# jarek1992/raytracer_project

Hardware: AMD Instinct MI355X
Metric: Msamples/sec (rays·bounces) (higher is better)
Workload: dtype f64

## Files before the change

### raytracer_project_amd/csrc/zr_build.hip

```cpp
#include <cstring>
#include <hip/hip_runtime.h>
#include <rocprim/device/device_radix_sort.hpp>
#include <rocprim/device/device_scan.hpp>
#include <rocprim/iterator/counting_iterator.hpp>
#include <rocprim/iterator/transform_iterator.hpp>

#include <algorithm>
#include <chrono>
#include <cstdio>
#include <vector>

#include "zr_build.h"
#include "zr_bvh.h"

namespace zr {
namespace {

constexpr uint32_t NONE = 0xFFFFFFFFu;
constexpr int MAX_R = 32;
constexpr uint32_t M_KIND = 7u, M_UNIFORM = 8u, M_LEAF = 16u;

struct PBox { float lo[3]; uint32_t kind; float hi[3]; uint32_t pad; };
struct Cl { float lo[3]; uint32_t node; float hi[3]; uint32_t pad; };
struct BNode { float lo[3]; uint32_t left; float hi[3]; uint32_t right; };
// ... 346 lines not shown
    const uint32_t p = parent[id];
    if (p != NONE && (nmeta[p] & M_LEAF)) return;
    leaf_pos[id] = out.base[nmeta[id] & M_KIND] + rank[leaf_pos[id]];
}

__device__ __forceinline__ void plane_sum(float origin, float scale, int q, double& s, double& e) {
    const double a = (double)origin, m = (double)q * (double)scale;
    s = a + m;
    const double bb = s - a;
    e = (a - (s - bb)) + (m - bb);
}
__device__ __forceinline__ bool plane_le(float origin, float scale, int q, double x) { double s, e; plane_sum(origin, scale, q, s, e); return s < x || (s == x && e <= 0.0); }
__device__ __forceinline__ bool plane_ge(float origin, float scale, int q, double x) { double s, e; plane_sum(origin, scale, q, s, e); return s > x || (s == x && e >= 0.0); }
__device__ __forceinline__ double plane_val(float origin, float scale, int q) { return (double)origin + (double)q * (double)scale; }

__device__ bool quant_axis(const float* lo, const float* hi, int n, float& origin, float& scale, uint32_t* qlo, uint32_t* qhi) {
    float mn = lo[0], mx = hi[0];
    for (int k = 1; k < n; k++) { mn = fminf(mn, lo[k]); mx = fmaxf(mx, hi[k]); }
    if (!(fabsf(mn) <= 1e30f) || !(fabsf(mx) <= 1e30f)) return false;
    origin = nextafterf(mn, -__builtin_huge_valf());
    const double ext = (double)mx - (double)origin;
    int e = ext > 0 ? (int)ceil(log2(ext / 255.0)) : -100;
    const int emin = origin != 0.0f ? max(-100, ilogbf(origin) - 30) : -100;
    if (e < emin) e = emin;
    for (int tries = 0; tries < 64; tries++, e++) {
        scale = ldexpf(1.0f, e);
        bool ok = true;
        for (int k = 0; k < n && ok; k++) {
            long ql = (long)floor(((double)lo[k] - (double)origin) / (double)scale);
            ql = ql < 0 ? 0 : (ql > 255 ? 255 : ql);
            while (ql > 0 && !plane_le(origin, scale, (int)ql, (double)lo[k])) ql--;
            if (!plane_le(origin, scale, (int)ql, (double)lo[k])) ok = false;
            long qh = (long)ceil(((double)hi[k] - (double)origin) / (double)scale);
            qh = qh < 0 ? 0 : (qh > 255 ? 255 : qh);
            while (qh < 255 && !plane_ge(origin, scale, (int)qh, (double)hi[k])) qh++;
            if (!plane_ge(origin, scale, (int)qh, (double)hi[k])) ok = false;
            qlo[k] = (uint32_t)ql; qhi[k] = (uint32_t)qh;
        }
        if (ok) return true;
    }
    return false;
}

__device__ bool quantise(const BNode* __restrict__ bn, const uint32_t* kids, int nk, NodeQ& nq, float& worst) {
    uint32_t ql[3][4], qh[3][4];
    for (int k = 0; k < 6; k++) nq.q[k] = 0;
    for (int ax = 0; ax < 3; ax++) {
        float lo[4], hi[4];
        for (int k = 0; k < nk; k++) { lo[k] = bn[kids[k]].lo[ax]; hi[k] = bn[kids[k]].hi[ax]; }
        if (!quant_axis(lo, hi, nk, nq.origin[ax], nq.scale[ax], ql[ax], qh[ax])) return false;
        for (int k = 0; k < nk; k++) { nq.q[ax] |= ql[ax][k] << (8 * k); nq.q[3 + ax] |= qh[ax][k] << (8 * k); }
    }
    worst = 1;
    for (int k = 0; k < nk; k++) {
        double d[3];
        for (int ax = 0; ax < 3; ax++) d[ax] = plane_val(nq.origin[ax], nq.scale[ax], (int)qh[ax][k]) - plane_val(nq.origin[ax], nq.scale[ax], (int)ql[ax][k]);
        const double aq = d[0] * d[1] + d[1] * d[2] + d[2] * d[0];
        const BNode b = bn[kids[k]];
        const double at = (double)half_area(b.lo, b.hi);
        const float rr = at > 0 ? (float)(aq / at) : (aq > 0 ? 3.0e38f : 1.0f);
        if (!(rr <= worst)) worst = rr;
    }
    return true;
}

struct PlanOut {
    uint32_t counter;
    uint32_t quant_fail;
    uint32_t quad_depth;
    uint32_t kept_closed;
    uint32_t root_demand;
    uint32_t pad_[3];
    NodeF root;
};

__device__ __forceinline__ uint32_t leaf_ref(const uint32_t* __restrict__ nmeta, const uint32_t* __restrict__ ncount, const uint32_t* __restrict__ leaf_pos, uint32_t node) {
    return ZR_REF_LEAF | ((nmeta[node] & M_KIND) << 28) | ((ncount[node] - 1u) << 24) | leaf_pos[node];
}

__global__ __launch_bounds__(256) void k_plan(const BNode* __restrict__ bn, const uint32_t* __restrict__ nmeta, const uint32_t* __restrict__ ncount,
                                              const uint32_t* __restrict__ leaf_pos, uint32_t node_lo, uint32_t node_hi, uint32_t root, int root_in_array, float open_ratio,
                                              const zr_object* __restrict__ objs, const uint32_t* __restrict__ run_demand,
                                              uint32_t* __restrict__ qroot, uint32_t* __restrict__ qlevel, uint32_t* __restrict__ qinst, NodeQ* __restrict__ quads,
                                              PlanOut* __restrict__ po) {
    const uint32_t id = node_lo + blockIdx.x * 256 + threadIdx.x;
    if (id >= node_hi) return;
    const bool is_root = id == root;
    const bool fp32_root = is_root && !root_in_array;
    const uint32_t me = qroot[id];
    if (!fp32_root && me == NONE) return;
    uint32_t kids[4]; int nk = 0;
    NodeQ nq;
    for (int ax = 0; ax < 3; ax++) { nq.origin[ax] = 0; nq.scale[ax] = 1; }
    for (int k = 0; k < 6; k++) nq.q[k] = 0;
    float worst = 1;
    if (nmeta[id] & M_LEAF) {
        kids[nk++] = id;
        if (!fp32_root && !quantise(bn, kids, nk, nq, worst)) atomicExch(&po->quant_fail, 1u);
    } else {
        const BNode b = bn[id];
        kids[0] = b.left; kids[1] = b.right; nk = 2;
        if (!fp32_root && !quantise(bn, kids, nk, nq, worst)) atomicExch(&po->quant_fail, 1u);
        while (nk < 4) {
            int best = -1; float ba = -1;
            for (int k = 0; k < nk; k++) {
                if (nmeta[kids[k]] & M_LEAF) continue;
                const BNode c = bn[kids[k]];
                const float ar = half_area(c.lo, c.hi);
                if (ar > ba) { ba = ar; best = k; }
            }
            if (best < 0) break;
            uint32_t trial[4];
            for (int k = 0; k < nk; k++) trial[k] = kids[k];
            const BNode ob = bn[kids[best]];
            trial[best] = ob.left; trial[nk] = ob.right;
            if (!fp32_root) {
                NodeQ tq = nq; float w = 1;
                if (!quantise(bn, trial, nk + 1, tq, w)) { atomicExch(&po->quant_fail, 1u); break; }
                if (w > open_ratio && w > worst) { atomicAdd(&po->kept_closed, 1u); break; }
                nq = tq; worst = w;
            }
            for (int k = 0; k <= nk; k++) kids[k] = trial[k];
            nk++;
        }
    }
    int n_inner = 0;
    for (int k = 0; k < nk; k++) if (!(nmeta[kids[k]] & M_LEAF)) n_inner++;
    uint32_t next = n_inner ? atomicAdd(&po->counter, (uint32_t)n_inner) : 0u;
    const uint32_t my_level = fp32_root ? 0u : qlevel[me];
    uint32_t refs[4] = {ZR_REF_EMPTY, ZR_REF_EMPTY, ZR_REF_EMPTY, ZR_REF_EMPTY};
    uint32_t inst_demand = 0;
    for (int k = 0; k < nk; k++) {
        const uint32_t c = kids[k];
        if (nmeta[c] & M_LEAF) {
            refs[k] = leaf_ref(nmeta, ncount, leaf_pos, c);
            if ((nmeta[c] & M_KIND) == ZR_KIND_INSTANCE && run_demand && objs) {
                uint32_t q = c;
                while (bn[q].right != NONE) q = bn[q].left;
// ... 229 lines not shown

}

DeviceBuilder::~DeviceBuilder() {
    if (arena_) (void)hipFree(arena_);
    for (void* p : keep_) (void)hipFree(p);
}
void* DeviceBuilder::alloc_keep(size_t bytes) {
    void* p = nullptr;
    if (hipMalloc(&p, bytes < 64 ? 64 : bytes) != hipSuccess) { (void)hipGetLastError(); return nullptr; }
    keep_.push_back(p);
    return p;
}
size_t DeviceBuilder::scratch_bytes(uint32_t n) {
    const size_t N = 2 * (size_t)n + 2;
    return (size_t)n * (32 + 16 + 8 + 64 + 4 + 1 + 4 + 1 + 4 + 4 + 4 + 4 + 4 + 4 + 8) + N * (32 + 4 + 4 + 4 + 4 + 4 + 4) + (size_t)n * 24 + (64u << 20);
}
hipError_t DeviceBuilder::reserve(size_t bytes) {
    if (bytes <= arena_bytes_) return hipSuccess;
    if (arena_) { (void)hipStreamSynchronize(st_); (void)hipFree(arena_); arena_ = nullptr; arena_bytes_ = 0; }
    hipError_t e = hipMalloc((void**)&arena_, bytes);
    if (e != hipSuccess) { (void)hipGetLastError(); err_ = "out of device memory for the build's scratch"; return e; }
    arena_bytes_ = bytes;
    return hipSuccess;
}

hipError_t DeviceBuilder::build(const BuildSceneIn& in, const zr_object* d_objects, const uint8_t* d_code, uint32_t first_triangle, uint32_t n,
                                const BuildParams& bp, bool root_in_array, const BuildPrimOut& out, const uint32_t* d_run_demand, uint32_t depth_limit,
                                bool stats, BuiltTree& t) {
    hipError_t e;
    err_ = ""; use_host_ = false;
    if (n == 0) { err_ = "empty tree"; use_host_ = true; return hipErrorInvalidValue; }
    Params prm;
    prm.ct = bp.ct; prm.max_leaf = bp.max_leaf < 1 ? 1 : (bp.max_leaf > 16 ? 16 : bp.max_leaf); prm.open_ratio = bp.open_ratio;
    prm.radius = bp.radius < 1 ? 1 : (bp.radius > MAX_R ? MAX_R : bp.radius);
    for (int k = 0; k < 8; k++) { prm.ck[k] = bp.ck[k]; prm.cap[k] = bp.leaf_cap[k]; }
    const size_t N = 2 * (size_t)n;
    const uint32_t nb_max = (n + 255) / 256;
    PBox* pbox; uint64_t *keys_a, *keys_b; uint32_t *vals_a, *vals_b; Cl *cl_a, *cl_b; BNode* bn;
    uint32_t *parent, *ncount, *nmeta, *leaf_pos, *qroot, *nn, *blk_keep, *blk_new, *keep_off, *new_off, *dfs_obj, *rank, *scanned, *qlevel, *qinst, *qdem, *compound, *state;
    float* ncost; uint8_t *act, *dfs_kind; PlanOut* po; void* tmp; size_t tmp_bytes = 0;
    uint32_t *qinst_plan, *qmap, *qscan; NodeQ* quads_plan;
    auto layout = [&](unsigned char* base) -> size_t {
        unsigned char* at = base;
        auto take = [&](size_t bytes) { void* p = at; at += (bytes + 255) / 256 * 256; return p; };
        pbox = (PBox*)take((size_t)n * sizeof(PBox));
        keys_a = (uint64_t*)take((size_t)n * 8); keys_b = (uint64_t*)take((size_t)n * 8);
        vals_a = (uint32_t*)take((size_t)n * 4); vals_b = (uint32_t*)take((size_t)n * 4);
        cl_a = (Cl*)take((size_t)n * sizeof(Cl)); cl_b = (Cl*)take((size_t)n * sizeof(Cl));
        bn = (BNode*)take(N * sizeof(BNode));
        parent = (uint32_t*)take(N * 4); ncount = (uint32_t*)take(N * 4); nmeta = (uint32_t*)take(N * 4);
        ncost = (float*)take(N * 4);
        leaf_pos = (uint32_t*)take(N * 4); qroot = (uint32_t*)take(N * 4);
        nn = (uint32_t*)take((size_t)n * 4); act = (uint8_t*)take(n);
        blk_keep = (uint32_t*)take((size_t)nb_max * 4); blk_new = (uint32_t*)take((size_t)nb_max * 4);
        keep_off = (uint32_t*)take((size_t)nb_max * 4); new_off = (uint32_t*)take((size_t)nb_max * 4);
        dfs_obj = (uint32_t*)take((size_t)n * 4); dfs_kind = (uint8_t*)take(n);
        rank = (uint32_t*)take((size_t)n * 4); scanned = (uint32_t*)take((size_t)n * 4);
        qlevel = (uint32_t*)take((size_t)n * 4); qinst = (uint32_t*)take((size_t)n * 4); qdem = (uint32_t*)take((size_t)n * 4);
        qinst_plan = (uint32_t*)take((size_t)n * 4); qmap = (uint32_t*)take((size_t)n * 4); qscan = (uint32_t*)take(N * 4);
        quads_plan = (NodeQ*)take((size_t)n * sizeof(NodeQ));
        compound = (uint32_t*)take((size_t)n * 8);
        state = (uint32_t*)take(256);
        po = (PlanOut*)take(sizeof(PlanOut));
        if (tmp_bytes == 0) {
            size_t a = 0, b = 0, c = 0;
            (void)rocprim::radix_sort_pairs(nullptr, a, keys_a, keys_b, vals_a, vals_b, (size_t)n, 0, 63, st_);
            (void)rocprim::exclusive_scan(nullptr, b, rocprim::make_transform_iterator(dfs_kind, IsKind{0}), scanned, 0u, (size_t)n, rocprim::plus<uint32_t>(), st_);
// ... 143 lines not shown
    if ((e = hipMemsetAsync(qinst, 0, (size_t)n * 4, st_)) != hipSuccess) return e;
    if ((e = hipMemsetAsync(qdem, 0, (size_t)n * 4, st_)) != hipSuccess) return e;
    auto renumber = [&]() -> hipError_t {
        auto flags = rocprim::make_transform_iterator(rocprim::make_counting_iterator<uint32_t>(0u), QRootFlag{qroot, root});
        hipError_t er = rocprim::exclusive_scan(tmp, tmp_bytes, flags, qscan, 0u, (size_t)n_nodes, rocprim::plus<uint32_t>(), st_);
        if (er != hipSuccess) { err_ = "scan failed"; return er; }
        hipLaunchKernelGGL(k_qmap, grid_for(n_nodes), dim3(256), 0, st_, qroot, qscan, n_nodes, qmap);
        hipLaunchKernelGGL(k_qpermute, grid_for(quad_cap), dim3(256), 0, st_, quads_plan, quads, qinst_plan, qinst, qmap, quad_cap, po);
        return hipSuccess;
    };
    if (root_in_array) {
        if ((e = hipMemsetAsync(qroot + root, 0, 4, st_)) != hipSuccess) return e;
        if ((e = hipMemsetAsync(qlevel, 0, 4, st_)) != hipSuccess) return e;
    }
    if (n == 1) {
        hipLaunchKernelGGL(k_plan, dim3(1), dim3(256), 0, st_, bn, nmeta, ncount, leaf_pos, root, root + 1, root, root_in_array ? 1 : 0, prm.open_ratio, d_objects, d_run_demand,
                           qroot, qlevel, qinst_plan, quads_plan, po);
        if ((e = renumber()) != hipSuccess) return e;
        hipLaunchKernelGGL(k_demand, dim3(1), dim3(256), 0, st_, qroot, root, root + 1, root, root_in_array ? 1 : 0, quads, qinst, qdem, po);
    } else {
        for (size_t b = batch_start.size() - 1; b-- > 0;) {
            const uint32_t lo = batch_start[b], hi = batch_start[b + 1];
            hipLaunchKernelGGL(k_plan, grid_for(hi - lo), dim3(256), 0, st_, bn, nmeta, ncount, leaf_pos, lo, hi, root, root_in_array ? 1 : 0, prm.open_ratio, d_objects,
                               d_run_demand, qroot, qlevel, qinst_plan, quads_plan, po);
        }
        if ((e = renumber()) != hipSuccess) return e;
        for (size_t b = 0; b + 1 < batch_start.size(); b++) {
            const uint32_t lo = batch_start[b], hi = batch_start[b + 1];
            hipLaunchKernelGGL(k_demand, grid_for(hi - lo), dim3(256), 0, st_, qroot, lo, hi, root, root_in_array ? 1 : 0, quads, qinst, qdem, po);
        }
    }
    lap(4);
    uint32_t n_pairs = 1;
    if (n >= 2) {
        uint32_t h_root_meta = 0;
        if ((e = hipMemcpyAsync(&h_root_meta, nmeta + root, 4, hipMemcpyDeviceToHost, st_)) != hipSuccess) return e;
        if ((e = hipStreamSynchronize(st_)) != hipSuccess) return e;
        if (h_root_meta & M_LEAF) hipLaunchKernelGGL(k_pair_leaf_root, dim3(1), dim3(1), 0, st_, bn, nmeta, ncount, leaf_pos, root, pairs);
// ... 44 lines not shown
```

### raytracer_project_amd/csrc/zr_commit.cpp

```cpp
#include "zr_flatten.h"

namespace {

int finish_commit(zr_scene* s, const CommitSummary& cs, size_t n_objs) {
    int rc;
    if (std::getenv("ZR_QUANT_STATS")) std::fprintf(stderr, "[zr] 4-wide nodes: %zu quantised (64 B) + FP32 root; %zu children kept closed for the grid\n", cs.n_quads, cs.kept_closed);
    s->quad_ok = cs.quant_ok && cs.n_quads < (1u << 31) && cs.max_leaf <= 16 && cs.n_sph < (1u << 24) && cs.n_tri < (1u << 24) && cs.n_cube < (1u << 24) &&
                 cs.n_media < (1u << 24) && cs.n_wrapped < (1u << 24) && cs.n_pcube < (1u << 24) && cs.n_insts < (1u << 24);
    if ((rc = s->d_ops.upload(s->ops.data(), s->ops.size()))) return rc;
    {
        std::vector<zr_material> mats = s->materials;
        auto tex_uses_uv = [&](uint32_t id) {
            std::vector<uint32_t> todo{id}; int guard = 0;
            while (!todo.empty() && guard++ < 4096) {
                uint32_t t = todo.back(); todo.pop_back();
                if (t >= s->textures.size()) continue;
                const zr_texture& tx = s->textures[t];
                if (tx.kind >= ZR_TEX_IMAGE_U8) return true;
                if (tx.kind == ZR_TEX_CHECKER) { todo.push_back(tx.odd); todo.push_back(tx.even); }
            }
            return guard >= 4096;
        };
        for (zr_material& m : mats) m.pad_ = (m.bump_tex != ZR_NO_TEXTURE || (m.kind != ZR_MAT_DIELECTRIC && tex_uses_uv(m.tex))) ? 1u : 0u;
        if ((rc = s->d_mats.upload(mats))) return rc;
// ... 215 lines not shown
            hipError_t e = builder->build(in, nullptr, nullptr, grp.first_triangle, grp.triangle_count, bp, true, go, nullptr, ZR_STACK_DEPTH - 2, false, runs[g]);
            if (e != hipSuccess) return build_fail(e);
            for (int k = 0; k < 6; k++) gbox[g * 6 + k] = runs[g].box[k];
            run_demand[g] = runs[g].demand;
        }
    }
    if (ng) { if ((rc = r_gbox.upload(gbox)) || (rc = d_run_demand.upload(run_demand))) return rc; in.group_box = r_gbox.p; }
    phase("groups' trees");
    zr::BuiltTree world;
    world.want_boxes = std::getenv("ZR_BUILD_CHECK") != nullptr;
    {
        hipError_t e = builder->build(in, r_objs.p, r_code.p, 0, n, bp, false, out, ng ? d_run_demand.p : nullptr, ZR_STACK_DEPTH - 2, commit_stats, world);
        if (e != hipSuccess) return build_fail(e);
    }
    if (commit_stats)
        std::fprintf(stderr, "[zr] device build: boxes+keys %.2f, sort %.2f, PLOC %.2f (%u iterations), order %.2f, 4-wide %.2f, pairs %.2f, emit %.2f ms; depth %u, %u pairs, %u quads\n",
                     world.ms[0], world.ms[1], world.ms[2], world.ploc_iterations, world.ms[3], world.ms[4], world.ms[5], world.ms[6], world.depth, world.n_pairs, world.n_quads);
    if (world.want_boxes) {
        std::vector<zr::BuildBox> gb(ng);
        for (size_t g = 0; g < ng; g++) for (int k = 0; k < 3; k++) { gb[g].lo[k] = gbox[g * 6 + k]; gb[g].hi[k] = gbox[g * 6 + 3 + k]; }
        Boxer boxer{*s, &gb};
        size_t bad = 0;
        for (uint32_t k = 0; k < n; k++) {
            const zr::BuildBox hb = boxer.chain(objs[k].type, objs[k].index, objs[k].chain_first, objs[k].chain_count);
            const float* d = &world.dbg_boxes[(size_t)k * 8];
            bool ok = true;
            for (int a = 0; a < 3; a++) if (!((double)d[a] <= hb.lo[a]) || !((double)d[4 + a] >= hb.hi[a])) ok = false;
            if (!ok && bad++ < 8)
                std::fprintf(stderr, "[zr] BUILD_CHECK: object %u (type %u, chain %u): device box [%g %g %g | %g %g %g] does not contain the host's [%g %g %g | %g %g %g]\n", k, objs[k].type,
                             objs[k].chain_count, d[0], d[1], d[2], d[4], d[5], d[6], hb.lo[0], hb.lo[1], hb.lo[2], hb.hi[0], hb.hi[1], hb.hi[2]);
        }
        if (bad) return fail(ZR_E_DEVICE, "ZR_BUILD_CHECK: %zu of %u object boxes computed on the device do not contain the host's", bad, n);
// ... 290 lines not shown
                    env_double("ZR_BVH_COST_MEDIUM", 3.0), env_double("ZR_BVH_COST_WRAPPED", 3.0), env_double("ZR_BVH_COST_PCUBE", 1.5),
                    env_double("ZR_BVH_COST_GROUP", 16.0), 1};
    int max_leaf = (int)env_double("ZR_BVH_MAX_LEAF", 4);
    const int big = (int)env_double("ZR_BVH_MAX_LEAF_BIG", 1);
    const int leaf_cap[8] = {0, 0, big, big, big, big, 1, 0};
    phase("boxes");
    zr::build_bvh(boxes, kinds, max_leaf, ZR_STACK_DEPTH - 2, env_double("ZR_BVH_COST_TRAVERSE", 1.0), ck, br, leaf_cap);
    phase("binned-SAH build");
    if (br.max_depth >= ZR_STACK_DEPTH - 1) return fail(ZR_E_INVALID, "BVH depth %d exceeds the traversal stack", br.max_depth);

    std::shared_ptr<Flattener> flp(new Flattener{*s, objs, br});
    Flattener& fl = *flp;
    fl.baked = &baked;
    fl.runs = runs.empty() ? nullptr : &runs;
    fl.open_ratio = env_double("ZR_BVH_OPEN_RATIO", 1.25);
    fl.want_src = true;
    int up_rc = ZR_OK;
    std::string up_err;
    std::thread uploader;
    const int device = s->ctx ? s->ctx->device : 0;
    fl.after_primitives = [&]() {
        uploader = std::thread([&, device]() {
            auto go = [&]() -> int {
                HIP_OK(hipSetDevice(device));
                int r;
                if ((r = s->d_spheres.upload(fl.spheres))) return r;
                if ((r = s->d_sphere_mat.upload(fl.sphere_mat))) return r;
                if ((r = s->d_tri_v.upload(fl.tri_v))) return r;
                if ((r = s->d_tri_s.upload(fl.tri_s))) return r;
                if ((r = s->d_cubes.upload(fl.cubes))) return r;
// ... 123 lines not shown
```

### raytracer_project_amd/csrc/zr_flatten.h

```cpp
#pragma once
#include "zr_host_internal.h"

namespace {

struct Boxer {
    const zr_scene& s;
    const std::vector<zr::BuildBox>* group_box = nullptr;
    zr::BuildBox prim(uint32_t type, uint32_t idx) const {
        zr::BuildBox b;
        if (type == ZR_PRIM_GROUP) return (*group_box)[idx];
        if (type == ZR_PRIM_SPHERE) {
            const double* q = &s.spheres[(size_t)idx * 4];
            for (int k = 0; k < 3; k++) { b.lo[k] = std::fmin(q[k] - q[3], q[k] + q[3]); b.hi[k] = std::fmax(q[k] - q[3], q[k] + q[3]); }
        } else if (type == ZR_PRIM_TRIANGLE) {
            const double* v = &s.tri_v[(size_t)idx * 9];
            for (int k = 0; k < 3; k++) {
                b.lo[k] = std::fmin(v[k], std::fmin(v[3 + k], v[6 + k]));
                b.hi[k] = std::fmax(v[k], std::fmax(v[3 + k], v[6 + k]));
                if (b.hi[k] - b.lo[k] < 0.0001) { b.lo[k] -= 0.0001; b.hi[k] += 0.0001; }
            }
        } else if (type == ZR_PRIM_CUBE) {
            const double* q = &s.cubes[(size_t)idx * 12];
            for (int k = 0; k < 3; k++) { b.lo[k] = q[6 + k] - 0.00005; b.hi[k] = q[9 + k] + 0.00005; }
        } else {
// ... 432 lines not shown
        return dx * dy + dy * dz + dz * dx;
    }
    static long double plane(float origin, float scale, long q) { return (long double)origin + (long double)q * (long double)scale; }
    static bool quant_axis(const double* lo, const double* hi, int n, float& origin, float& scale, uint8_t* qlo, uint8_t* qhi) {
        double mn = lo[0], mx = hi[0];
        for (int k = 1; k < n; k++) { mn = std::min(mn, lo[k]); mx = std::max(mx, hi[k]); }
        if (!std::isfinite(mn) || !std::isfinite(mx) || std::fabs(mn) > 1e30 || std::fabs(mx) > 1e30) return false;
        origin = f_down(mn);
        const double ext = mx - (double)origin;
        int e = ext > 0 ? (int)std::ceil(std::log2(ext / 255.0)) : -100;
        const int emin = origin != 0.0f ? std::max(-100, std::ilogb(origin) - 30) : -100;
        if (e < emin) e = emin;
        for (int tries = 0; tries < 64; tries++, e++) {
            scale = std::ldexp(1.0f, e);
            bool ok = true;
            for (int k = 0; k < n && ok; k++) {
                long ql = (long)std::floor((lo[k] - (double)origin) / (double)scale);
                ql = std::min(255l, std::max(0l, ql));
                while (ql > 0 && plane(origin, scale, ql) > (long double)lo[k]) ql--;
                if (plane(origin, scale, ql) > (long double)lo[k]) ok = false;
                long qh = (long)std::ceil((hi[k] - (double)origin) / (double)scale);
                qh = std::min(255l, std::max(0l, qh));
                while (qh < 255 && plane(origin, scale, qh) < (long double)hi[k]) qh++;
                if (plane(origin, scale, qh) < (long double)hi[k]) ok = false;
                qlo[k] = (uint8_t)ql; qhi[k] = (uint8_t)qh;
            }
            if (ok) return true;
        }
        return false;
    }
    double open_ratio = 1.25;
    zr::NodeF root{};
    size_t n_kept_closed = 0;
    bool quantise(const int32_t* kids, int nk, zr::NodeQ& nq, double* worst) const {
        uint8_t ql[3][4] = {}, qh[3][4] = {};
        for (int k = 0; k < 6; k++) nq.q[k] = 0;
        for (int ax = 0; ax < 3; ax++) {
            double lo[4], hi[4];
            for (int k = 0; k < nk; k++) { lo[k] = br.nodes[kids[k]].box.lo[ax]; hi[k] = br.nodes[kids[k]].box.hi[ax]; }
            if (!quant_axis(lo, hi, nk, nq.origin[ax], nq.scale[ax], ql[ax], qh[ax])) return false;
            for (int k = 0; k < nk; k++) { nq.q[ax] |= (uint32_t)ql[ax][k] << (8 * k); nq.q[3 + ax] |= (uint32_t)qh[ax][k] << (8 * k); }
        }
        *worst = 1;
        for (int k = 0; k < nk; k++) {
// ... 1 lines not shown
            for (int ax = 0; ax < 3; ax++) {
                qb.lo[ax] = (double)plane(nq.origin[ax], nq.scale[ax], ql[ax][k]);
                qb.hi[ax] = (double)plane(nq.origin[ax], nq.scale[ax], qh[ax][k]);
            }
            const double at = area(br.nodes[kids[k]].box), aq = area(qb);
            const double r = at > 0 ? aq / at : (aq > 0 ? 1e300 : 1.0);
            if (!(r <= *worst)) *worst = r;
        }
        return true;
    }
    std::atomic<bool> quant_ok_a{true};
    bool quant_ok = true;
    std::atomic<size_t> kept_closed_a{0};
    struct QuadPlan { int32_t kids[4]; int nk; zr::NodeQ nq; };
    zr::RawArray<QuadPlan> plan;
    void plan_quad(int32_t node_id, bool is_root, QuadPlan& qp) const {
        int32_t* kids = qp.kids; int nk = 0;
        zr::NodeQ nq{};
        for (int ax = 0; ax < 3; ax++) nq.scale[ax] = 1;
        if (br.nodes[node_id].count) kids[nk++] = node_id;
        else {
            nk = 2;
            kids[0] = br.nodes[node_id].left; kids[1] = br.nodes[node_id].right;
            double worst = 1;
            if (!is_root && !quantise(kids, nk, nq, &worst)) const_cast<Flattener*>(this)->quant_ok_a = false;
            while (nk < 4) {
                int best = -1; double ba = -1;
                for (int k = 0; k < nk; k++) if (br.nodes[kids[k]].count == 0 && area(br.nodes[kids[k]].box) > ba) { ba = area(br.nodes[kids[k]].box); best = k; }
                if (best < 0) break;
                int32_t trial[4];
                for (int k = 0; k < nk; k++) trial[k] = kids[k];
                trial[best] = br.nodes[kids[best]].left; trial[nk] = br.nodes[kids[best]].right;
                if (!is_root) {
                    zr::NodeQ tq = nq; double w = 1;
                    if (!quantise(trial, nk + 1, tq, &w)) { const_cast<Flattener*>(this)->quant_ok_a = false; break; }
                    if (w > open_ratio && w > worst) { const_cast<Flattener*>(this)->kept_closed_a++; break; }
                    nq = tq; worst = w;
                }
                for (int k = 0; k <= nk; k++) kids[k] = trial[k];
                nk++;
            }
        }
        qp.nk = nk; qp.nq = nq;
    }
    std::vector<std::vector<int32_t>> levels;
    zr::RawArray<uint32_t> q_size, q_index;
    void plan_quads(int32_t root_id) {
        plan.allocate(br.nodes.size());
        levels.clear();
        levels.push_back(std::vector<int32_t>{root_id});
        bool first = !root_in_array;
        for (;;) {
            const std::vector<int32_t>& level = levels.back();
            const int T = std::max(1, threads);
            std::vector<std::vector<int32_t>> out((size_t)T);
            std::atomic<int> slot{0};
            parallel_for(level.size(), 256, [&](size_t a2, size_t b2) {
                std::vector<int32_t>& mine = out[(size_t)slot.fetch_add(1)];
                for (size_t i = a2; i < b2; i++) {
                    QuadPlan& qp = plan[level[i]];
                    plan_quad(level[i], first, qp);
                    for (int k = 0; k < qp.nk; k++) if (br.nodes[qp.kids[k]].count == 0) mine.push_back(qp.kids[k]);
// ... 164 lines not shown
            parallel_for(inner.size(), 4096, [&](size_t a, size_t b) { for (size_t p = a; p < b; p++) fill_pair((uint32_t)p, inner[p]); });
        }
        ph("pair records");
        plan_quads(0);
        ph("4-wide plan");
        number_quads(0);
        ph("4-wide numbering");
        if (runs) { emit_run_quads(); ph("groups' 4-wide nodes"); }
    }
    void emit_run_quads() {
        run_qroot.assign(runs->size(), 0); run_demand.assign(runs->size(), 0);
        const std::vector<zr_object> none;
        for (size_t g = 0; g < runs->size(); g++) {
            const zr::BuildResult& rb = (*runs)[g];
            Flattener sub{s, none, rb};
            sub.threads = 1; sub.open_ratio = open_ratio; sub.root_in_array = true;
            sub.leaf_first.allocate(rb.nodes.size()); sub.pair_of.allocate(rb.nodes.size());
            const uint32_t base = (uint32_t)quads.size();
            run_qroot[g] = base;
            if (rb.nodes[0].count) {
                zr::NodeQ nq{};
                int32_t kid = 0; double w = 1;
                for (int ax = 0; ax < 3; ax++) nq.scale[ax] = 1;
                if (!sub.quantise(&kid, 1, nq, &w)) quant_ok_a = false;
                for (int k = 0; k < 4; k++) nq.ref[k] = ZR_REF_EMPTY;
                nq.ref[0] = ZR_REF_LEAF | ((uint32_t)ZR_PRIM_TRIANGLE << 28) | ((uint32_t)(rb.nodes[0].count - 1u) << 24) | run_tri_base[g];
                quads.push_back(nq);
                run_demand[g] = 1;
                continue;
            }
            sub.index_nodes();
// ... 9 lines not shown
                quads.push_back(nq);
            }
            run_demand[g] = sub.demand_of(sub.quads[0].ref) + 0u;
        }
        quant_ok = quant_ok && quant_ok_a.load();
        for (size_t i = 0; i < insts.size(); i++) insts[i].pad_ = run_qroot[inst_group[i]];
    }
    void fill_leaf_root() {
        const zr::BuildNode& n = br.nodes[0];
        for (int k = 0; k < 3; k++) { pairs[0].lo[0][k] = f_down(n.box.lo[k]); pairs[0].hi[0][k] = f_up(n.box.hi[k]); }
        pairs[0].child[0] = leaf_first[0]; pairs[0].meta[0] = ((n.kind + 1u) << 16) | n.count;
        empty_child(0, 1);
    }
};

}
```

Baseline: 5866.

## Collapse binary BVH to 4-wide nodes with bottom-up SAH dynamic programming

Replaces the greedy largest-area child-opening rule with a bottom-up dynamic program. It runs on both the device and host builders and picks, for each inner node, the cut of its binary subtree (up to depth 3) into at most four children that minimises SAH cost. The cost uses the quantised child areas and per-primitive-kind cost weights, and respects a bound on quantisation blow-up. The aim is a 4-wide tree with lower expected traversal cost, so rendering throughput improves. It adds a collapse pass with its own per-node cost and cut buffers, and new cost statistics output.

After: 5898, median of 6. No clear change (+0.5%).

```diff
diff --git a/raytracer_project_amd/csrc/zr_build.hip b/raytracer_project_amd/csrc/zr_build.hip
--- a/raytracer_project_amd/csrc/zr_build.hip
+++ b/raytracer_project_amd/csrc/zr_build.hip
@@ -384,6 +384,19 @@
 __device__ __forceinline__ bool plane_ge(float origin, float scale, int q, double x) { double s, e; plane_sum(origin, scale, q, s, e); return s > x || (s == x && e >= 0.0); }
 __device__ __forceinline__ double plane_val(float origin, float scale, int q) { return (double)origin + (double)q * (double)scale; }
 
+__device__ __forceinline__ bool quant_one(float origin, float scale, float lo, float hi, uint32_t& qlo, uint32_t& qhi) {
+    bool ok = true;
+    long ql = (long)floor(((double)lo - (double)origin) / (double)scale);
+    ql = ql < 0 ? 0 : (ql > 255 ? 255 : ql);
+    while (ql > 0 && !plane_le(origin, scale, (int)ql, (double)lo)) ql--;
+    if (!plane_le(origin, scale, (int)ql, (double)lo)) ok = false;
+    long qh = (long)ceil(((double)hi - (double)origin) / (double)scale);
+    qh = qh < 0 ? 0 : (qh > 255 ? 255 : qh);
+    while (qh < 255 && !plane_ge(origin, scale, (int)qh, (double)hi)) qh++;
+    if (!plane_ge(origin, scale, (int)qh, (double)hi)) ok = false;
+    qlo = (uint32_t)ql; qhi = (uint32_t)qh;
+    return ok;
+}
 __device__ bool quant_axis(const float* lo, const float* hi, int n, float& origin, float& scale, uint32_t* qlo, uint32_t* qhi) {
     float mn = lo[0], mx = hi[0];
     for (int k = 1; k < n; k++) { mn = fminf(mn, lo[k]); mx = fmaxf(mx, hi[k]); }
@@ -396,17 +409,7 @@
     for (int tries = 0; tries < 64; tries++, e++) {
         scale = ldexpf(1.0f, e);
         bool ok = true;
-        for (int k = 0; k < n && ok; k++) {
-            long ql = (long)floor(((double)lo[k] - (double)origin) / (double)scale);
-            ql = ql < 0 ? 0 : (ql > 255 ? 255 : ql);
-            while (ql > 0 && !plane_le(origin, scale, (int)ql, (double)lo[k])) ql--;
-            if (!plane_le(origin, scale, (int)ql, (double)lo[k])) ok = false;
-            long qh = (long)ceil(((double)hi[k] - (double)origin) / (double)scale);
-            qh = qh < 0 ? 0 : (qh > 255 ? 255 : qh);
-            while (qh < 255 && !plane_ge(origin, scale, (int)qh, (double)hi[k])) qh++;
-            if (!plane_ge(origin, scale, (int)qh, (double)hi[k])) ok = false;
-            qlo[k] = (uint32_t)ql; qhi[k] = (uint32_t)qh;
-        }
+        for (int k = 0; k < n && ok; k++) ok = quant_one(origin, scale, lo[k], hi[k], qlo[k], qhi[k]);
         if (ok) return true;
     }
     return false;
@@ -434,6 +437,90 @@
     return true;
 }
 
+constexpr int CUT_SLOTS = 15;
+__device__ __forceinline__ double grid_area(const float* origin, const float* scale, const uint32_t* ql, const uint32_t* qh) {
+    double d[3];
+    for (int ax = 0; ax < 3; ax++) d[ax] = plane_val(origin[ax], scale[ax], (int)qh[ax]) - plane_val(origin[ax], scale[ax], (int)ql[ax]);
+    return d[0] * d[1] + d[1] * d[2] + d[2] * d[0];
+}
+__global__ __launch_bounds__(256) void k_collapse(const BNode* __restrict__ bn, const uint32_t* __restrict__ nmeta, const uint32_t* __restrict__ ncount, uint32_t node_lo,
+                                                  uint32_t node_hi, uint32_t root, int root_in_array, Params prm, float* __restrict__ vcost, uint8_t* __restrict__ cut) {
+    const uint32_t id = node_lo + blockIdx.x * 256 + threadIdx.x;
+    if (id >= node_hi || (nmeta[id] & M_LEAF)) return;
+    const bool fp32_root = id == root && !root_in_array;
+    uint32_t node[CUT_SLOTS]; bool inner[CUT_SLOTS];
+    node[0] = id; inner[0] = true;
+#pragma unroll
+    for (int i = 1; i < CUT_SLOTS; i++) {
+        const int p = (i - 1) / 2;
+        node[i] = NONE; inner[i] = false;
+        if (node[p] != NONE && inner[p]) { const BNode b = bn[node[p]]; node[i] = (i & 1) ? b.left : b.right; inner[i] = !(nmeta[node[i]] & M_LEAF); }
+    }
+    float origin[3] = {0, 0, 0}, scale[3] = {1, 1, 1};
+    bool grid = !fp32_root;
+    if (grid) {
+        const BNode l = bn[node[1]], r = bn[node[2]];
+        for (int ax = 0; ax < 3 && grid; ax++) {
+            const float lo[2] = {l.lo[ax], r.lo[ax]}, hi[2] = {l.hi[ax], r.hi[ax]};
+            uint32_t ql[2], qh[2];
+            grid = quant_axis(lo, hi, 2, origin[ax], scale[ax], ql, qh);
+        }
+    }
+    float w[CUT_SLOTS], rr[CUT_SLOTS];
+#pragma unroll
+    for (int i = 1; i < CUT_SLOTS; i++) {
+        w[i] = __builtin_huge_valf(); rr[i] = __builtin_huge_valf();
+        if (node[i] == NONE) continue;
+        const BNode c = bn[node[i]];
+        const double at = (double)half_area(c.lo, c.hi);
+        double aq = at;
+        if (fp32_root) rr[i] = 1;
+        else if (grid) {
+            uint32_t ql[3], qh[3];
+            bool ok = true;
+            for (int ax = 0; ax < 3; ax++) ok = quant_one(origin[ax], scale[ax], c.lo[ax], c.hi[ax], ql[ax], qh[ax]) && ok;
+            if (ok) { aq = grid_area(origin, scale, ql, qh); rr[i] = at > 0 ? (float)(aq / at) : (aq > 0 ? 3.0e38f : 1.0f); }
+        } else if (i <= 2) rr[i] = 1;
+        const float sub = inner[i] ? vcost[node[i]] : prm.ck[nmeta[node[i]] & M_KIND] * (float)ncount[node[i]];
+        w[i] = (float)aq * sub;
+    }
+    const float bound = fmaxf(prm.open_ratio, fmaxf(rr[1], rr[2]));
+    float best[CUT_SLOTS][4]; uint8_t split[7][4];
+#pragma unroll
+    for (int i = CUT_SLOTS - 1; i >= 1; i--) {
+        best[i][0] = rr[i] <= bound ? w[i] : __builtin_huge_valf();
+        const bool can_open = i <= 6 && inner[i];
+#pragma unroll
+        for (int k = 2; k <= 4; k++) {
+            float v = best[i][k - 2]; uint8_t sp = 0;
+            if (can_open) {
+#pragma unroll
+                for (int j = 1; j < k; j++) { const float c = best[2 * i + 1][j - 1] + best[2 * i + 2][k - j - 1]; if (c < v) { v = c; sp = (uint8_t)j; } }
+            }
+            best[i][k - 1] = v;
+            if (i <= 6) split[i][k - 1] = sp;
+        }
+    }
+    float total = __builtin_huge_valf(); int j0 = 1;
+#pragma unroll
+    for (int j = 1; j <= 3; j++) { const float c = best[1][j - 1] + best[2][3 - j]; if (c < total) { total = c; j0 = j; } }
+    int kk[CUT_SLOTS];
+#pragma unroll
+    for (int i = 0; i < CUT_SLOTS; i++) kk[i] = 0;
+    kk[1] = j0; kk[2] = 4 - j0;
+    uint32_t mask = 0;
+#pragma unroll
+    for (int i = 1; i <= 6; i++) {
+        int k = kk[i];
+        while (k > 1 && split[i][k - 1] == 0) k--;
+        if (k > 1) { mask |= 1u << (i - 1); const int j = split[i][k - 1]; kk[2 * i + 1] = j; kk[2 * i + 2] = k - j; }
+    }
+    const BNode me = bn[id];
+    const double an = (double)half_area(me.lo, me.hi);
+    vcost[id] = prm.ct + (float)((double)total / (an > 0 ? an : 1.0));
+    cut[id] = (uint8_t)mask;
+}
+
 struct PlanOut {
     uint32_t counter;
     uint32_t quant_fail;
@@ -449,8 +536,8 @@
 }
 
 __global__ __launch_bounds__(256) void k_plan(const BNode* __restrict__ bn, const uint32_t* __restrict__ nmeta, const uint32_t* __restrict__ ncount,
-                                              const uint32_t* __restrict__ leaf_pos, uint32_t node_lo, uint32_t node_hi, uint32_t root, int root_in_array, float open_ratio,
-                                              const zr_object* __restrict__ objs, const uint32_t* __restrict__ run_demand,
+                                              const uint32_t* __restrict__ leaf_pos, const uint8_t* __restrict__ cut, uint32_t node_lo, uint32_t node_hi, uint32_t root,
+                                              int root_in_array, const zr_object* __restrict__ objs, const uint32_t* __restrict__ run_demand,
                                               uint32_t* __restrict__ qroot, uint32_t* __restrict__ qlevel, uint32_t* __restrict__ qinst, NodeQ* __restrict__ quads,
                                               PlanOut* __restrict__ po) {
     const uint32_t id = node_lo + blockIdx.x * 256 + threadIdx.x;
@@ -468,30 +555,25 @@
         kids[nk++] = id;
         if (!fp32_root && !quantise(bn, kids, nk, nq, worst)) atomicExch(&po->quant_fail, 1u);
     } else {
+        const uint32_t mask = cut[id];
         const BNode b = bn[id];
-        kids[0] = b.left; kids[1] = b.right; nk = 2;
-        if (!fp32_root && !quantise(bn, kids, nk, nq, worst)) atomicExch(&po->quant_fail, 1u);
-        while (nk < 4) {
-            int best = -1; float ba = -1;
-            for (int k = 0; k < nk; k++) {
-                if (nmeta[kids[k]] & M_LEAF) continue;
-                const BNode c = bn[kids[k]];
-                const float ar = half_area(c.lo, c.hi);
-                if (ar > ba) { ba = ar; best = k; }
+        const uint32_t d1[2] = {b.left, b.right};
+        for (int a = 0; a < 2; a++) {
+            if (!(mask & (1u << a))) { kids[nk++] = d1[a]; continue; }
+            const BNode ba = bn[d1[a]];
+            const uint32_t d2[2] = {ba.left, ba.right};
+            for (int c = 0; c < 2; c++) {
+                const int slot = 3 + 2 * a + c;
+                if (!(mask & (1u << (slot - 1)))) { kids[nk++] = d2[c]; continue; }
+                const BNode bc = bn[d2[c]];
+                kids[nk++] = bc.left; kids[nk++] = bc.right;
             }
-            if (best < 0) break;
-            uint32_t trial[4];
-            for (int k = 0; k < nk; k++) trial[k] = kids[k];
-            const BNode ob = bn[kids[best]];
-            trial[best] = ob.left; trial[nk] = ob.right;
-            if (!fp32_root) {
-                NodeQ tq = nq; float w = 1;
-                if (!quantise(bn, trial, nk + 1, tq, w)) { atomicExch(&po->quant_fail, 1u); break; }
-                if (w > open_ratio && w > worst) { atomicAdd(&po->kept_closed, 1u); break; }
-                nq = tq; worst = w;
-            }
-            for (int k = 0; k <= nk; k++) kids[k] = trial[k];
-            nk++;
+        }
+        if (!fp32_root) {
+            if (!quantise(bn, kids, nk, nq, worst)) atomicExch(&po->quant_fail, 1u);
+            bool inner_kid = false;
+            for (int k = 0; k < nk; k++) if (!(nmeta[kids[k]] & M_LEAF)) inner_kid = true;
+            if (nk < 4 && inner_kid) atomicAdd(&po->kept_closed, 1u);
         }
     }
     int n_inner = 0;
@@ -751,7 +833,7 @@
 }
 size_t DeviceBuilder::scratch_bytes(uint32_t n) {
     const size_t N = 2 * (size_t)n + 2;
-    return (size_t)n * (32 + 16 + 8 + 64 + 4 + 1 + 4 + 1 + 4 + 4 + 4 + 4 + 4 + 4 + 8) + N * (32 + 4 + 4 + 4 + 4 + 4 + 4) + (size_t)n * 24 + (64u << 20);
+    return (size_t)n * (32 + 16 + 8 + 64 + 4 + 1 + 4 + 1 + 4 + 4 + 4 + 4 + 4 + 4 + 8) + N * (32 + 4 + 4 + 4 + 4 + 4 + 4 + 4 + 1) + (size_t)n * 24 + (64u << 20);
 }
 hipError_t DeviceBuilder::reserve(size_t bytes) {
     if (bytes <= arena_bytes_) return hipSuccess;
@@ -776,7 +858,7 @@
     const uint32_t nb_max = (n + 255) / 256;
     PBox* pbox; uint64_t *keys_a, *keys_b; uint32_t *vals_a, *vals_b; Cl *cl_a, *cl_b; BNode* bn;
     uint32_t *parent, *ncount, *nmeta, *leaf_pos, *qroot, *nn, *blk_keep, *blk_new, *keep_off, *new_off, *dfs_obj, *rank, *scanned, *qlevel, *qinst, *qdem, *compound, *state;
-    float* ncost; uint8_t *act, *dfs_kind; PlanOut* po; void* tmp; size_t tmp_bytes = 0;
+    float *ncost, *vcost; uint8_t *act, *dfs_kind, *cut; PlanOut* po; void* tmp; size_t tmp_bytes = 0;
     uint32_t *qinst_plan, *qmap, *qscan; NodeQ* quads_plan;
     auto layout = [&](unsigned char* base) -> size_t {
         unsigned char* at = base;
@@ -789,6 +871,7 @@
         parent = (uint32_t*)take(N * 4); ncount = (uint32_t*)take(N * 4); nmeta = (uint32_t*)take(N * 4);
         ncost = (float*)take(N * 4);
         leaf_pos = (uint32_t*)take(N * 4); qroot = (uint32_t*)take(N * 4);
+        vcost = (float*)take(N * 4); cut = (uint8_t*)take(N);
         nn = (uint32_t*)take((size_t)n * 4); act = (uint8_t*)take(n);
         blk_keep = (uint32_t*)take((size_t)nb_max * 4); blk_new = (uint32_t*)take((size_t)nb_max * 4);
         keep_off = (uint32_t*)take((size_t)nb_max * 4); new_off = (uint32_t*)take((size_t)nb_max * 4);
@@ -962,14 +1045,19 @@
         if ((e = hipMemsetAsync(qlevel, 0, 4, st_)) != hipSuccess) return e;
     }
     if (n == 1) {
-        hipLaunchKernelGGL(k_plan, dim3(1), dim3(256), 0, st_, bn, nmeta, ncount, leaf_pos, root, root + 1, root, root_in_array ? 1 : 0, prm.open_ratio, d_objects, d_run_demand,
+        hipLaunchKernelGGL(k_plan, dim3(1), dim3(256), 0, st_, bn, nmeta, ncount, leaf_pos, cut, root, root + 1, root, root_in_array ? 1 : 0, d_objects, d_run_demand,
                            qroot, qlevel, qinst_plan, quads_plan, po);
         if ((e = renumber()) != hipSuccess) return e;
         hipLaunchKernelGGL(k_demand, dim3(1), dim3(256), 0, st_, qroot, root, root + 1, root, root_in_array ? 1 : 0, quads, qinst, qdem, po);
     } else {
+        for (size_t b = 0; b + 1 < batch_start.size(); b++) {
+            const uint32_t lo = batch_start[b], hi = batch_start[b + 1];
+            hipLaunchKernelGGL(k_collapse, grid_for(hi - lo), dim3(256), 0, st_, bn, nmeta, ncount, lo, hi, root, root_in_array ? 1 : 0, prm, vcost, cut);
+        }
+        lap(7);
         for (size_t b = batch_start.size() - 1; b-- > 0;) {
             const uint32_t lo = batch_start[b], hi = batch_start[b + 1];
-            hipLaunchKernelGGL(k_plan, grid_for(hi - lo), dim3(256), 0, st_, bn, nmeta, ncount, leaf_pos, lo, hi, root, root_in_array ? 1 : 0, prm.open_ratio, d_objects,
+            hipLaunchKernelGGL(k_plan, grid_for(hi - lo), dim3(256), 0, st_, bn, nmeta, ncount, leaf_pos, cut, lo, hi, root, root_in_array ? 1 : 0, d_objects,
                                d_run_demand, qroot, qlevel, qinst_plan, quads_plan, po);
         }
         if ((e = renumber()) != hipSuccess) return e;
diff --git a/raytracer_project_amd/csrc/zr_commit.cpp b/raytracer_project_amd/csrc/zr_commit.cpp
--- a/raytracer_project_amd/csrc/zr_commit.cpp
+++ b/raytracer_project_amd/csrc/zr_commit.cpp
@@ -4,7 +4,18 @@
 
 int finish_commit(zr_scene* s, const CommitSummary& cs, size_t n_objs) {
     int rc;
-    if (std::getenv("ZR_QUANT_STATS")) std::fprintf(stderr, "[zr] 4-wide nodes: %zu quantised (64 B) + FP32 root; %zu children kept closed for the grid\n", cs.n_quads, cs.kept_closed);
+    if (std::getenv("ZR_QUANT_STATS")) {
+        std::fprintf(stderr, "[zr] 4-wide nodes: %zu quantised (64 B) + FP32 root; %zu nodes with an inner child and fewer than 4 children (the grid's bound)\n", cs.n_quads,
+                     cs.kept_closed);
+        std::vector<zr::NodeQ> hq(cs.n_quads);
+        if (!hq.empty() && hipMemcpy(hq.data(), s->d_quads.p, hq.size() * sizeof(zr::NodeQ), hipMemcpyDeviceToHost) != hipSuccess) { (void)hipGetLastError(); hq.clear(); }
+        const double ck[8] = {env_double("ZR_BVH_COST_SPHERE", 1.0), env_double("ZR_BVH_COST_TRI", 1.5), env_double("ZR_BVH_COST_CUBE", 1.0),
+                              env_double("ZR_BVH_COST_MEDIUM", 3.0), env_double("ZR_BVH_COST_WRAPPED", 3.0), env_double("ZR_BVH_COST_PCUBE", 1.5),
+                              env_double("ZR_BVH_COST_GROUP", 16.0), 1};
+        const TreeCost tc = quad_tree_cost(cs.root, hq, env_double("ZR_BVH_COST_TRAVERSE", 1.0), ck);
+        std::fprintf(stderr, "[zr] 4-wide tree cost (%s): SAH below the root's inner children %.4f; per root child %.4f %.4f %.4f %.4f (%zu %zu %zu %zu nodes); "
+                     "%zu inner children, %zu leaf children, %zu empty slots\n", cs.builder, tc.below, tc.sah[0], tc.sah[1], tc.sah[2], tc.sah[3], tc.nodes[0], tc.nodes[1], tc.nodes[2], tc.nodes[3], tc.inner, tc.leaves, tc.empty);
+    }
     s->quad_ok = cs.quant_ok && cs.n_quads < (1u << 31) && cs.max_leaf <= 16 && cs.n_sph < (1u << 24) && cs.n_tri < (1u << 24) && cs.n_cube < (1u << 24) &&
                  cs.n_media < (1u << 24) && cs.n_wrapped < (1u << 24) && cs.n_pcube < (1u << 24) && cs.n_insts < (1u << 24);
     if ((rc = s->d_ops.upload(s->ops.data(), s->ops.size()))) return rc;
@@ -253,8 +264,9 @@
         if (e != hipSuccess) return build_fail(e);
     }
     if (commit_stats)
-        std::fprintf(stderr, "[zr] device build: boxes+keys %.2f, sort %.2f, PLOC %.2f (%u iterations), order %.2f, 4-wide %.2f, pairs %.2f, emit %.2f ms; depth %u, %u pairs, %u quads\n",
-                     world.ms[0], world.ms[1], world.ms[2], world.ploc_iterations, world.ms[3], world.ms[4], world.ms[5], world.ms[6], world.depth, world.n_pairs, world.n_quads);
+        std::fprintf(stderr, "[zr] device build: boxes+keys %.2f, sort %.2f, PLOC %.2f (%u iterations), order %.2f, 4-wide collapse %.2f, 4-wide plan %.2f, pairs %.2f, emit %.2f ms; "
+                     "depth %u, %u pairs, %u quads\n", world.ms[0], world.ms[1], world.ms[2], world.ploc_iterations, world.ms[3], world.ms[7], world.ms[4], world.ms[5], world.ms[6],
+                     world.depth, world.n_pairs, world.n_quads);
     if (world.want_boxes) {
         std::vector<zr::BuildBox> gb(ng);
         for (size_t g = 0; g < ng; g++) for (int k = 0; k < 3; k++) { gb[g].lo[k] = gbox[g * 6 + k]; gb[g].hi[k] = gbox[g * 6 + 3 + k]; }
@@ -575,6 +587,8 @@
     fl.baked = &baked;
     fl.runs = runs.empty() ? nullptr : &runs;
     fl.open_ratio = env_double("ZR_BVH_OPEN_RATIO", 1.25);
+    fl.ct = env_double("ZR_BVH_COST_TRAVERSE", 1.0);
+    for (int k = 0; k < 8; k++) fl.ck[k] = ck[k];
     fl.want_src = true;
     int up_rc = ZR_OK;
     std::string up_err;
diff --git a/raytracer_project_amd/csrc/zr_flatten.h b/raytracer_project_amd/csrc/zr_flatten.h
--- a/raytracer_project_amd/csrc/zr_flatten.h
+++ b/raytracer_project_amd/csrc/zr_flatten.h
@@ -470,20 +470,23 @@
         for (int tries = 0; tries < 64; tries++, e++) {
             scale = std::ldexp(1.0f, e);
             bool ok = true;
-            for (int k = 0; k < n && ok; k++) {
-                long ql = (long)std::floor((lo[k] - (double)origin) / (double)scale);
-                ql = std::min(255l, std::max(0l, ql));
-                while (ql > 0 && plane(origin, scale, ql) > (long double)lo[k]) ql--;
-                if (plane(origin, scale, ql) > (long double)lo[k]) ok = false;
-                long qh = (long)std::ceil((hi[k] - (double)origin) / (double)scale);
-                qh = std::min(255l, std::max(0l, qh));
-                while (qh < 255 && plane(origin, scale, qh) < (long double)hi[k]) qh++;
-                if (plane(origin, scale, qh) < (long double)hi[k]) ok = false;
-                qlo[k] = (uint8_t)ql; qhi[k] = (uint8_t)qh;
-            }
+            for (int k = 0; k < n && ok; k++) ok = quant_one(origin, scale, lo[k], hi[k], qlo[k], qhi[k]);
             if (ok) return true;
         }
         return false;
+    }
+    static bool quant_one(float origin, float scale, double lo, double hi, uint8_t& qlo, uint8_t& qhi) {
+        bool ok = true;
+        long ql = (long)std::floor((lo - (double)origin) / (double)scale);
+        ql = std::min(255l, std::max(0l, ql));
+        while (ql > 0 && plane(origin, scale, ql) > (long double)lo) ql--;
+        if (plane(origin, scale, ql) > (long double)lo) ok = false;
+        long qh = (long)std::ceil((hi - (double)origin) / (double)scale);
+        qh = std::min(255l, std::max(0l, qh));
+        while (qh < 255 && plane(origin, scale, qh) < (long double)hi) qh++;
+        if (plane(origin, scale, qh) < (long double)hi) ok = false;
+        qlo = (uint8_t)ql; qhi = (uint8_t)qh;
+        return ok;
     }
     double open_ratio = 1.25;
     zr::NodeF root{};
@@ -515,31 +518,101 @@
     std::atomic<size_t> kept_closed_a{0};
     struct QuadPlan { int32_t kids[4]; int nk; zr::NodeQ nq; };
     zr::RawArray<QuadPlan> plan;
+    double ct = 1.0;
+    double ck[8] = {1, 1.5, 1, 3, 3, 1.5, 16, 1};
+    zr::RawArray<double> vcost;
+    zr::RawArray<uint8_t> cut;
+    void collapse_node(int32_t id, bool fp32_root) {
+        constexpr int S = 15;
+        const double inf = std::numeric_limits<double>::infinity();
+        int32_t node[S]; bool inn[S];
+        node[0] = id; inn[0] = true;
+        for (int i = 1; i < S; i++) {
+            const int p = (i - 1) / 2;
+            node[i] = -1; inn[i] = false;
+            if (node[p] >= 0 && inn[p]) { node[i] = (i & 1) ? br.nodes[node[p]].left : br.nodes[node[p]].right; inn[i] = br.nodes[node[i]].count == 0; }
+        }
+        float origin[3] = {0, 0, 0}, scale[3] = {1, 1, 1};
+        bool grid = !fp32_root;
+        for (int ax = 0; ax < 3 && grid; ax++) {
+            const double lo[2] = {br.nodes[node[1]].box.lo[ax], br.nodes[node[2]].box.lo[ax]}, hi[2] = {br.nodes[node[1]].box.hi[ax], br.nodes[node[2]].box.hi[ax]};
+            uint8_t ql[2], qh[2];
+            grid = quant_axis(lo, hi, 2, origin[ax], scale[ax], ql, qh);
+        }
+        double w[S], rr[S];
+        for (int i = 1; i < S; i++) {
+            w[i] = inf; rr[i] = inf;
+            if (node[i] < 0) continue;
+            const zr::BuildNode& c = br.nodes[node[i]];
+            const double at = area(c.box);
+            double aq = at;
+            if (fp32_root) rr[i] = 1;
+            else if (grid) {
+                uint8_t ql[3], qh[3];
+                bool ok = true;
+                for (int ax = 0; ax < 3; ax++) ok = quant_one(origin[ax], scale[ax], c.box.lo[ax], c.box.hi[ax], ql[ax], qh[ax]) && ok;
+                if (ok) {
+                    zr::BuildBox qb;
+                    for (int ax = 0; ax < 3; ax++) { qb.lo[ax] = (double)plane(origin[ax], scale[ax], ql[ax]); qb.hi[ax] = (double)plane(origin[ax], scale[ax], qh[ax]); }
+                    aq = area(qb);
+                    rr[i] = at > 0 ? aq / at : (aq > 0 ? 1e300 : 1.0);
+                }
+            } else if (i <= 2) rr[i] = 1;
+            w[i] = aq * (inn[i] ? vcost[node[i]] : ck[c.kind & 7] * (double)c.count);
+        }
+        const double bound = std::max(open_ratio, std::max(rr[1], rr[2]));
+        double best[S][4]; uint8_t split[7][4] = {};
+        for (int i = S - 1; i >= 1; i--) {
+            best[i][0] = rr[i] <= bound ? w[i] : inf;
+            for (int k = 2; k <= 4; k++) {
+                double v = best[i][k - 2]; uint8_t sp = 0;
+                if (i <= 6 && inn[i])
+                    for (int j = 1; j < k; j++) { const double c = best[2 * i + 1][j - 1] + best[2 * i + 2][k - j - 1]; if (c < v) { v = c; sp = (uint8_t)j; } }
+                best[i][k - 1] = v;
+                if (i <= 6) split[i][k - 1] = sp;
+            }
+        }
+        double total = inf; int j0 = 1;
+        for (int j = 1; j <= 3; j++) { const double c = best[1][j - 1] + best[2][3 - j]; if (c < total) { total = c; j0 = j; } }
+        int kk[S] = {};
+        kk[1] = j0; kk[2] = 4 - j0;
+        uint8_t mask = 0;
+        for (int i = 1; i <= 6; i++) {
+            int k = kk[i];
+            while (k > 1 && split[i][k - 1] == 0) k--;
+            if (k > 1) { mask |= (uint8_t)(1u << (i - 1)); const int j = split[i][k - 1]; kk[2 * i + 1] = j; kk[2 * i + 2] = k - j; }
+        }
+        const double an = area(br.nodes[id].box);
+        vcost[id] = ct + total / (an > 0 ? an : 1.0);
+        cut[id] = mask;
+    }
+    void collapse(int32_t root_id) {
+        vcost.allocate(br.nodes.size()); cut.allocate(br.nodes.size());
+        for (size_t i = inner.size(); i-- > 0;) collapse_node(inner[i], inner[i] == root_id && !root_in_array);
+    }
     void plan_quad(int32_t node_id, bool is_root, QuadPlan& qp) const {
         int32_t* kids = qp.kids; int nk = 0;
         zr::NodeQ nq{};
         for (int ax = 0; ax < 3; ax++) nq.scale[ax] = 1;
         if (br.nodes[node_id].count) kids[nk++] = node_id;
         else {
-            nk = 2;
-            kids[0] = br.nodes[node_id].left; kids[1] = br.nodes[node_id].right;
-            double worst = 1;
-            if (!is_root && !quantise(kids, nk, nq, &worst)) const_cast<Flattener*>(this)->quant_ok_a = false;
-            while (nk < 4) {
-                int best = -1; double ba = -1;
-                for (int k = 0; k < nk; k++) if (br.nodes[kids[k]].count == 0 && area(br.nodes[kids[k]].box) > ba) { ba = area(br.nodes[kids[k]].box); best = k; }
-                if (best < 0) break;
-                int32_t trial[4];
-                for (int k = 0; k < nk; k++) trial[k] = kids[k];
-                trial[best] = br.nodes[kids[best]].left; trial[nk] = br.nodes[kids[best]].right;
-                if (!is_root) {
-                    zr::NodeQ tq = nq; double w = 1;
-                    if (!quantise(trial, nk + 1, tq, &w)) { const_cast<Flattener*>(this)->quant_ok_a = false; break; }
-                    if (w > open_ratio && w > worst) { const_cast<Flattener*>(this)->kept_closed_a++; break; }
-                    nq = tq; worst = w;
-                }
-                for (int k = 0; k <= nk; k++) kids[k] = trial[k];
-                nk++;
+            const uint32_t mask = cut[node_id];
+            const int32_t d1[2] = {br.nodes[node_id].left, br.nodes[node_id].right};
+            for (int a = 0; a < 2; a++) {
+                if (!(mask & (1u << a))) { kids[nk++] = d1[a]; continue; }
+                const int32_t d2[2] = {br.nodes[d1[a]].left, br.nodes[d1[a]].right};
+                for (int c = 0; c < 2; c++) {
+                    const int slot = 3 + 2 * a + c;
+                    if (!(mask & (1u << (slot - 1)))) { kids[nk++] = d2[c]; continue; }
+                    kids[nk++] = br.nodes[d2[c]].left; kids[nk++] = br.nodes[d2[c]].right;
+                }
+            }
+            if (!is_root) {
+                double worst = 1;
+                if (!quantise(kids, nk, nq, &worst)) const_cast<Flattener*>(this)->quant_ok_a = false;
+                bool inner_kid = false;
+                for (int k = 0; k < nk; k++) if (br.nodes[kids[k]].count == 0) inner_kid = true;
+                if (nk < 4 && inner_kid) const_cast<Flattener*>(this)->kept_closed_a++;
             }
         }
         qp.nk = nk; qp.nq = nq;
@@ -547,6 +620,7 @@
     std::vector<std::vector<int32_t>> levels;
     zr::RawArray<uint32_t> q_size, q_index;
     void plan_quads(int32_t root_id) {
+        collapse(root_id);
         plan.allocate(br.nodes.size());
         levels.clear();
         levels.push_back(std::vector<int32_t>{root_id});
@@ -741,7 +815,8 @@
         for (size_t g = 0; g < runs->size(); g++) {
             const zr::BuildResult& rb = (*runs)[g];
             Flattener sub{s, none, rb};
-            sub.threads = 1; sub.open_ratio = open_ratio; sub.root_in_array = true;
+            sub.threads = 1; sub.open_ratio = open_ratio; sub.root_in_array = true; sub.ct = ct;
+            for (int k = 0; k < 8; k++) sub.ck[k] = ck[k];
             sub.leaf_first.allocate(rb.nodes.size()); sub.pair_of.allocate(rb.nodes.size());
             const uint32_t base = (uint32_t)quads.size();
             run_qroot[g] = base;
@@ -781,4 +856,47 @@
     }
 };
 
+struct TreeCost { double sah[4] = {0, 0, 0, 0}, below = 0; size_t nodes[4] = {0, 0, 0, 0}; size_t inner = 0, leaves = 0, empty = 0; };
+inline TreeCost quad_tree_cost(const zr::NodeF& root, const std::vector<zr::NodeQ>& quads, double ct, const double ck[8]) {
+    TreeCost tc;
+    auto harea = [](const double* lo, const double* hi) { const double dx = hi[0] - lo[0], dy = hi[1] - lo[1], dz = hi[2] - lo[2]; return dx * dy + dy * dz + dz * dx; };
+    std::vector<std::pair<uint32_t, double>> todo;
+    double sum = 0, below = 0, ulo[3] = {0, 0, 0}, uhi[3] = {0, 0, 0};
+    bool any = false;
+    auto child = [&](uint32_t ref, double a) {
+        if (ref == ZR_REF_EMPTY) { tc.empty++; return; }
+        if (ref & ZR_REF_LEAF) { tc.leaves++; sum += a * ck[(ref >> 28) & 7u] * (double)(((ref >> 24) & 15u) + 1u); return; }
+        tc.inner++;
+        if (ref < quads.size()) todo.emplace_back(ref, a);
+    };
+    for (int r = 0; r < 4; r++) {
+        const double lo[3] = {root.lox[r], root.loy[r], root.loz[r]}, hi[3] = {root.hix[r], root.hiy[r], root.hiz[r]};
+        const double ar = root.ref[r] == ZR_REF_EMPTY ? 0.0 : harea(lo, hi);
+        sum = 0;
+        child(root.ref[r], ar);
+        while (!todo.empty()) {
+            const auto [q, a] = todo.back(); todo.pop_back();
+            sum += ct * a; tc.nodes[r]++;
+            const zr::NodeQ& nq = quads[q];
+            for (int c = 0; c < 4; c++) {
+                double clo[3], chi[3];
+                for (int ax = 0; ax < 3; ax++) {
+                    clo[ax] = (double)nq.origin[ax] + (double)((nq.q[ax] >> (8 * c)) & 255u) * (double)nq.scale[ax];
+                    chi[ax] = (double)nq.origin[ax] + (double)((nq.q[3 + ax] >> (8 * c)) & 255u) * (double)nq.scale[ax];
+                }
+                child(nq.ref[c], nq.ref[c] == ZR_REF_EMPTY ? 0.0 : harea(clo, chi));
+            }
+        }
+        tc.sah[r] = ar > 0 ? sum / ar : 0.0;
+        if (root.ref[r] != ZR_REF_EMPTY && !(root.ref[r] & ZR_REF_LEAF)) {
+            below += sum;
+            for (int ax = 0; ax < 3; ax++) { ulo[ax] = any ? std::min(ulo[ax], lo[ax]) : lo[ax]; uhi[ax] = any ? std::max(uhi[ax], hi[ax]) : hi[ax]; }
+            any = true;
+        }
+    }
+    const double au = any ? harea(ulo, uhi) : 0.0;
+    tc.below = au > 0 ? below / au : 0.0;
+    return tc;
 }
+
+}
```
